# JiaweiXu8/AD-GS

Measured on AMD Instinct MI355X. Metric: fwd+bwd frames/s, higher is better.
Workload: dtype f32; 1 GPU; C3: 1000000 Gaussians, 1920x1280, SH deg 3, 8 dynamic objects, flow+semantic outputs, 1 camera/GPU/step; P=1000000, camera_pool=16 cameras / time stamps per GPU, cycled one per step (train.py:55-61), settle_steps=91, capacity_reruns=0, launch=eager, parallelism=single GPU, gradient_exchange=none, camera_streams=1

## Files before the change

### ad-gs_amd/adgs/_lib.py

```python
import contextlib
import ctypes
import os

_HERE = os.path.dirname(os.path.abspath(__file__))
PKG_ROOT = os.path.dirname(_HERE)
LIB_PATH = os.environ.get("ADGS_LIB") or os.path.join(PKG_ROOT, "lib", "libadgs_hip.so")

ALLOC_FN = ctypes.CFUNCTYPE(ctypes.c_void_p, ctypes.c_void_p, ctypes.c_size_t)

_lib = None

c_p = ctypes.c_void_p
c_i = ctypes.c_int
c_f = ctypes.c_float

SIGNATURES = {
    "adgs_last_error": (ctypes.c_char_p, []),
    "adgs_device_check": (c_i, []),
    "adgs_raster_forward": (c_i, [ALLOC_FN, c_p, ALLOC_FN, c_p, ALLOC_FN, c_p, c_i, c_i, c_i, c_i, c_p, c_i, c_i,
                                  c_p, c_p, c_p, c_p, c_p, c_p, c_p, c_f, c_p, c_p, c_p, c_p, c_p, c_f, c_f, c_i,
                                  c_p, c_p, c_p, c_p, c_p, c_i, c_p, c_i, c_p]),
    "adgs_raster_render": (c_i, [ALLOC_FN, c_p, ALLOC_FN, c_p, ALLOC_FN, c_p, c_i, c_i, c_i, c_i, c_p, c_i, c_i,
                                 c_p, c_p, c_p, c_p, c_p, c_p, c_p, c_f, c_p, c_p, c_p, c_p, c_p, c_f, c_f, c_i,
                                 c_p, c_p, c_p, c_p, c_p, c_i, c_p, c_i, c_p]),
# ... 112 lines not shown
    "adgs_tsdf_extract_count": (c_i, [c_p, c_p, c_p, c_f, c_p, c_p, c_p]),
    "adgs_tsdf_extract_emit": (c_i, [c_p, c_p, c_p, c_p, c_f, c_p, c_p, c_p, c_p, c_p, c_p, c_p]),
    "adgs_mesh_label_temp_bytes": (ctypes.c_size_t, [ctypes.c_longlong, ctypes.c_longlong]),
    "adgs_mesh_label": (c_i, [c_i, c_i, c_p, c_p, c_p, c_p, c_p]),
    "adgs_mesh_table": (c_i, [c_i, c_i, c_i, c_p, c_p, c_p, c_p, c_p, c_p, c_p, c_p, c_p]),
    "adgs_mesh_keep_temp_bytes": (ctypes.c_size_t, [ctypes.c_longlong, ctypes.c_longlong]),
    "adgs_mesh_keep_count": (c_i, [c_i, c_i, c_i, c_p, c_p, c_p, c_p, c_p, c_p]),
    "adgs_mesh_keep_emit": (c_i, [c_i, c_i, c_p, c_p, c_p, c_p, c_p, c_p, c_p, c_p, c_p, c_p, c_p]),
    "adgs_mesh_normals_temp_bytes": (ctypes.c_size_t, [ctypes.c_longlong, ctypes.c_longlong]),
    "adgs_mesh_vertex_normals": (c_i, [c_i, c_i, c_p, c_p, c_p, c_p, c_p]),
    "adgs_test_v2_published_entries": (ctypes.c_longlong, [c_p, c_i, c_i, c_p]),
    "adgs_test_v2_scanned_candidates": (ctypes.c_longlong, [c_p, c_i, c_i, c_p]),
    "adgs_test_v2_tile_counters": (ctypes.c_longlong, [c_p, c_i, c_i, c_p, c_p, ctypes.c_longlong, c_p]),
    "adgs_test_v2_blend_batches": (ctypes.c_longlong, [c_p, c_i, c_i, c_p]),
    "adgs_test_v2_cell_ranges": (ctypes.c_longlong, [c_p, c_i, c_i, c_p, ctypes.c_longlong, c_p]),
    "adgs_test_abi_sizeof": (ctypes.c_size_t, [c_i]),
    "adgs_test_set_capacity_hints": (None, [ctypes.c_longlong, ctypes.c_longlong]),
    "adgs_test_env_reads": (ctypes.c_ulonglong, []),
    "adgs_test_scramble_slab_bounds": (c_i, [ctypes.c_uint]),
    "adgs_test_scan_temp_bytes": (ctypes.c_size_t, [ctypes.c_size_t]),
    "adgs_test_exclusive_scan_u32": (c_i, [c_p, c_p, ctypes.c_size_t, c_p, c_p]),
    "adgs_test_sort_temp_bytes": (ctypes.c_size_t, [ctypes.c_size_t]),
    "adgs_test_sort_pairs_u64": (c_i, [c_p, c_p, c_p, c_p, ctypes.c_size_t, c_i, c_p, c_p]),
    "adgs_test_sort_pairs_u32": (c_i, [c_p, c_p, c_p, c_p, ctypes.c_size_t, c_i, c_p, c_p]),
    "adgs_test_bilagrid_path": (c_i, [c_i, c_i, c_i, c_i, c_i]),
    "adgs_test_deform_plan": (c_i, [c_p, c_i, c_i, c_i, c_p, c_p, c_p, c_p, c_p, c_p, c_p, c_p, c_p, c_p]),
}


class RasterOptions(ctypes.Structure):
# ... 114 lines not shown
```

### ad-gs_amd/csrc/api.hip

```cpp
#include "common.h"
#include "kernels.h"
#include "../../include/adgs_rasterizer.h"
#include "../../include/adgs_optim.h"

#include <atomic>
#include <chrono>
#include <mutex>
#include <vector>
#include <cstdlib>
#include <algorithm>
#include <cmath>
#include <cstring>

namespace adgs {

static thread_local std::string g_last_error;
struct FrameContext {
	adgs_frame_stats stats;
	size_t hint_cells, hint_fine;
	unsigned hint_max_cell_chunks;
	bool bucket_frame_pending;
	long long reruns;
	int last_order_hint;
	uint32_t* slab_bounds;
// ... 53 lines not shown
		b.list_unsorted = c.take<uint32_t>(R);
		b.keys = c.take<uint64_t>(R);
		b.keys_unsorted = c.take<uint64_t>(R);
		b.sort_temp = c.take<char>(sort_temp_bytes(R));
		if (bytes) *bytes = c.size();
		return b;
	}
};

struct GeomStateV2 {
	Splat* splats; uint8_t* clamped; uint32_t* cells_touched; uint32_t* offsets; uint32_t* fine_touched; uint4* dupinfo;
	float* gacc; float* sh0; char* scan_temp; unsigned long long* fine_total;
	float* ddir;
	uint32_t* counters; uint32_t* cell_start; uint2* cell_work; uint32_t* bounds; uint32_t* counts;
	static constexpr size_t COUNTER_WORDS = MAX_CELLS + 2 * SCAN_AUX_SLOTS + 8;
	uint32_t* cell_count() const { return counters; }
	unsigned long long* bucket_fine_total() const { return reinterpret_cast<unsigned long long*>(counters + MAX_CELLS); }
	uint32_t* d_counts() const { return counters + MAX_CELLS + 2 * SCAN_AUX_SLOTS; }
	static GeomStateV2 carve(char* chunk, size_t P, size_t* bytes, bool with_ddir, size_t ncells = 0) {
		Carver c(chunk); GeomStateV2 g;
		g.counters = c.take<uint32_t>(COUNTER_WORDS);
		g.cell_start = c.take<uint32_t>(MAX_CELLS + 1);
		g.cell_work = c.take<uint2>(MAX_CELLS + 1);
		g.splats = c.take<Splat>(P);
		g.gacc = c.take<float>(P * GACC_STRIDE);
		g.dupinfo = c.take<uint4>(P);
		g.clamped = c.take<uint8_t>(P);
		g.cells_touched = c.take<uint32_t>(P + 1);
		g.offsets = c.take<uint32_t>(P + 1);
		g.fine_touched = c.take<uint32_t>(P + 1);
		g.sh0 = c.take<float>(P * 3);
		g.fine_total = c.take<unsigned long long>(SCAN_AUX_SLOTS);
		g.scan_temp = c.take<char>(scan_temp_bytes(P + 1));
		g.ddir = with_ddir ? c.take<float>(P * 9) : nullptr;
		const size_t nc = std::min<size_t>(ncells, (size_t)MAX_CELLS + 1);
		g.bounds = c.take<uint32_t>(nc * SLAB_ROW);
		g.counts = c.take<uint32_t>(count_row_stride((int)((P + 255) / 256)) * nc);
		if (bytes) *bytes = c.size();
		return g;
	}
};
struct ImgStateV2 {
// ... 147 lines not shown
			entries.push_back(fresh);
			e = &entries.back();
		}
		e->view = view; e->proj = proj; e->W = W; e->H = H; e->tiles = tiles; e->stream = stream; e->captured = captured; e->used = ++clock; e->written = false; e->extra = extra;
		if (!reset_signature(e->buf, tiles, extra)) { e->view = nullptr; e->tiles = 0; (void)hipFree(e->buf); e->buf = nullptr; return nullptr; }
		return e;
	}
};
static OrderHints* order_hints() {
	constexpr int MAX_DEV = 64;
	static thread_local OrderHints hints[MAX_DEV];
	int dev = 0;
	if (hipGetDevice(&dev) != hipSuccess || dev < 0 || dev >= MAX_DEV) return nullptr;
	return &hints[dev];
}
struct FrameCfg { int v2; int cell_tiles; int ppl; int tile_order = 1; int sh_staging = 1; int timeline = 0; int order_ready = 0; int backwards = 0; int antialiasing = 0; };
static uint32_t frame_cfg_word(const FrameCfg& c) {
	return 0xAD600000u | ((uint32_t)(c.v2 & 1) << 19) | ((uint32_t)(c.tile_order & 1) << 18) | ((uint32_t)(c.sh_staging & 1) << 17) | ((uint32_t)(c.timeline & 1) << 16) |
	       ((uint32_t)(c.order_ready & 1) << 15) | ((uint32_t)(c.antialiasing & 1) << 14) |
	       ((uint32_t)(c.ppl & 0x3f) << 8) | (uint32_t)(c.cell_tiles & 0xff);
}
static bool frame_cfg_from_word(uint32_t w, FrameCfg* c) {
	if ((w & 0xFFF00000u) != 0xAD600000u) return false;
	*c = FrameCfg{ (int)((w >> 19) & 1u), (int)(w & 0xffu), (int)((w >> 8) & 0x3fu) };
	c->tile_order = (int)((w >> 18) & 1u); c->sh_staging = (int)((w >> 17) & 1u); c->timeline = (int)((w >> 16) & 1u); c->order_ready = (int)((w >> 15) & 1u);
	c->antialiasing = (int)((w >> 14) & 1u);
	return c->cell_tiles >= 1 && (c->ppl == 1 || c->ppl == 2 || c->ppl == 4);
}
struct FrameKey {
	const void* img; const void* geom; int W, H, P;
	bool operator==(const FrameKey& o) const { return img == o.img && geom == o.geom && W == o.W && H == o.H && P == o.P; }
};
static std::mutex g_cfg_mu;
static std::vector<std::pair<FrameKey, FrameCfg>> g_cfg_table;
static void remember_frame(const FrameKey& k, const FrameCfg& c) {
	std::lock_guard<std::mutex> lk(g_cfg_mu);
	for (auto it = g_cfg_table.begin(); it != g_cfg_table.end();) it = (it->first.img == k.img || it->first.geom == k.geom) ? g_cfg_table.erase(it) : it + 1;
	if (g_cfg_table.size() >= 256) g_cfg_table.erase(g_cfg_table.begin());
	g_cfg_table.emplace_back(k, c);
}
static int note_backward(const FrameKey& k) {
// ... 159 lines not shown
		const int wgy = (height + 4 * ppl - 1) / (4 * ppl);
		const size_t wtiles = (size_t)gx * wgy;
		ImgStateV2::carve(nullptr, npix, wtiles, ncells, &ib);
		char* ich = imageBuffer(imageUser, ib);
		if (!gch || !ich) { set_error("buffer allocator returned NULL"); return -1; }
		GeomStateV2 geom = GeomStateV2::carve(gch, P, nullptr, with_ddir, count_cells);
		ImgStateV2 img = ImgStateV2::carve(ich, npix, wtiles, ncells, nullptr);
		uint32_t frame_word = 0; bool order_tiles = false;
		{
			FrameCfg fcfg{ 1, cell_tiles, ppl };
			fcfg.antialiasing = antialiasing ? 1 : 0;
			fcfg.tile_order = env_int("ADGS_TILE_ORDER", 1) != 0; fcfg.sh_staging = env_str("ADGS_NO_SH_STAGING") == nullptr; fcfg.timeline = env_int("ADGS_TIMELINE_BWD", 0) != 0;
			order_tiles = wtiles >= 2048 && fcfg.tile_order;
			if (!training) order_tiles = false;
			fcfg.order_ready = order_tiles ? 1 : 0;
			if (training) remember_frame(FrameKey{ ich, gch, width, height, P }, fcfg);
			frame_word = frame_cfg_word(fcfg);
		}
		const int fwd_order_mode = env_int("ADGS_FWD_ORDER", 2);
		OrderHints::Entry* hint = nullptr;
		const uint32_t* hint_read = nullptr;
		const bool fwd_hint_wanted = wtiles >= 2048 && env_int("ADGS_TILE_ORDER", 1) != 0 && fwd_order_mode == 2;
		if (fwd_hint_wanted) {
			hipStreamCaptureStatus cs0 = hipStreamCaptureStatusNone;
			(void)hipStreamIsCapturing(stream, &cs0);
			if (OrderHints* oh = order_hints()) {
				const bool cap0 = cs0 == hipStreamCaptureStatusActive;
				hint = oh->find(viewmatrix, projmatrix, width, height, wtiles, stream, cap0);
				if (!hint && training) {
					hipStreamCaptureMode mode = hipStreamCaptureModeRelaxed;
// ... 12 lines not shown
		pa.means3D = means3D; pa.scales = scales; pa.scale_modifier = scale_modifier; pa.rotations = rotations;
		pa.opacities = opacities; pa.shs = shs; pa.cov3D_precomp = cov3D_precomp; pa.colors_precomp = colors_precomp;
		pa.flow_points = flow_points; pa.semantic = semantic;
		pa.view = viewmatrix; pa.proj = projmatrix; pa.campos = cam_pos;
		pa.W = width; pa.H = height; pa.gx = gx; pa.gy = gy;
		pa.tan_fovx = tan_fovx; pa.tan_fovy = tan_fovy;
		pa.focal_y = height / (2.0f * tan_fovy); pa.focal_x = width / (2.0f * tan_fovx);
		pa.inv_depth = inv_depth;
		pa.radii = radii; pa.splats = geom.splats; pa.cov3D = nullptr; pa.clamped = geom.clamped; pa.tiles_touched = geom.cells_touched;
		pa.v2 = 1; pa.dupinfo = geom.dupinfo; pa.fine_touched = geom.fine_touched; pa.cell_tiles = cell_tiles; pa.cgx = cgx; pa.cgy = cgy;
		memset(&pa.sh_src, 0, sizeof(pa.sh_src));
		pa.sh0 = geom.sh0; pa.gacc = training ? geom.gacc : nullptr; pa.fine_total = geom.fine_total;
		pa.bucket_count = nullptr;
		pa.cfg_word = img.header; pa.cfg_value = frame_word;
		pa.ddir = geom.ddir;
		pa.antialias = antialiasing ? 1 : 0;
		FramePrologue pro{ nullptr, 0, nullptr, nullptr, 0 };
		bool own_bounds = false, sample_bounds = false;
		if (buckets) {
			if (!fc->slab_bounds) {
				hipStreamCaptureStatus csb = hipStreamCaptureStatusNone;
				(void)hipStreamIsCapturing(stream, &csb);
				hipStreamCaptureMode mode = hipStreamCaptureModeRelaxed;
				if (csb == hipStreamCaptureStatusActive) (void)hipThreadExchangeStreamCaptureMode(&mode);
				bool ok = hipMalloc((void**)&fc->slab_bounds, (size_t)MAX_CELLS * SLAB_ROW * sizeof(uint32_t)) == hipSuccess;
				ok = ok && (fc->service || hipStreamCreateWithFlags(&fc->service, hipStreamNonBlocking) == hipSuccess);
				ok = ok && hipMemsetAsync(fc->slab_bounds, 0xff, (size_t)MAX_CELLS * SLAB_ROW * sizeof(uint32_t), fc->service) == hipSuccess && hipStreamSynchronize(fc->service) == hipSuccess;
				if (csb == hipStreamCaptureStatusActive) (void)hipThreadExchangeStreamCaptureMode(&mode);
				if (!ok) { if (fc->slab_bounds) (void)hipFree(fc->slab_bounds); fc->slab_bounds = nullptr; (void)hipGetLastError(); }
			}
// ... 99 lines not shown
		};
		auto launch_blend = [&]() -> int {
			RenderV2FwdArgs ra;
			ra.cell_ranges = img.cell_ranges; ra.cell_list = bin.list; ra.splats = geom.splats;
			ra.cell_keys = bin.keys; ra.mask_shift = mask_shift; ra.cell_entries = buckets ? bin.entries : nullptr;
			ra.W = width; ra.H = height; ra.gx = gx; ra.gy = wgy; ra.ppl = ppl; ra.cell_tiles = cell_tiles; ra.cgx = cgx;
			ra.has_color = (colors_precomp != nullptr) || (shs != nullptr) || (sh_src != nullptr);
			ra.has_flow = flow_points != nullptr; ra.has_sem = (semantic != nullptr) && D_S > 0;
			ra.bg = background; ra.bg_image = sh_src ? sh_src->bg_image : nullptr;
			ra.pool = bin.pool; ra.pool_cursor = bin.pool_cursor; ra.tile_last_chunk = img.tile_last_chunk; ra.tile_consumed = img.tile_consumed; ra.tile_scanned = img.tile_scanned; ra.tile_batches = img.tile_batches;
			ra.final_T = img_opacity; ra.n_contrib = img.n_contrib;
			ra.out_color = out_color; ra.out_depth = out_depth; ra.out_flow = img_flow; ra.out_semantic = img_semantic;
			ra.order_mode = fwd_order_mode == 2 ? 1 : fwd_order_mode; ra.fwd_order = nullptr;
			ra.fwd_view = viewmatrix; ra.fwd_sig = nullptr;
			if (hint_read) { ra.order_mode = 2; ra.fwd_order = hint_read; ra.fwd_sig = reinterpret_cast<const float*>(hint_read + wtiles); }
			ra.overflow_flag = overflow_flag; ra.publish = training;
			{ StageTimer t(ST_RENDER_FWD, stream);
			  if (launch_render_fwd_v2(ra, stream) != 0) return -1;
			  for (int c0 = 1; ra.has_sem && c0 < D_S; c0 += 4) {
				RenderV2SemFwdArgs sa;
				sa.splats = geom.splats; sa.pool = bin.pool; sa.tile_last_chunk = img.tile_last_chunk; sa.tile_consumed = img.tile_consumed; sa.n_contrib = img.n_contrib;
				sa.W = width; sa.H = height; sa.gx = gx; sa.gy = wgy; sa.ppl = ppl;
				sa.semantic = semantic; sa.D_S = D_S; sa.c0 = c0; sa.nch = std::min(4, D_S - c0); sa.out_semantic = img_semantic;
				if (launch_render_sem_fwd_v2(sa, stream) != 0) return -1;
			  } }
			if (order_tiles) {
				StageTimer t(ST_RENDER_FWD, stream);
				if (launch_tile_order((int)wtiles, img.tile_consumed, img.tile_order, stream, hint ? hint->buf : nullptr, viewmatrix) != 0) return -1;
				if (hint) hint->written = true;
			}
			ADGS_LAUNCH_CHECK(debug, stream);
// ... 61 lines not shown
	PreprocessArgs pa;
	pa.P = P; pa.D = D; pa.M = M; pa.D_S = D_S;
	pa.means3D = means3D; pa.scales = scales; pa.scale_modifier = scale_modifier; pa.rotations = rotations;
	pa.opacities = opacities; pa.shs = shs; pa.cov3D_precomp = cov3D_precomp; pa.colors_precomp = colors_precomp;
	pa.flow_points = flow_points; pa.semantic = semantic;
	pa.view = viewmatrix; pa.proj = projmatrix; pa.campos = cam_pos;
	pa.W = width; pa.H = height; pa.gx = gx; pa.gy = gy;
	pa.tan_fovx = tan_fovx; pa.tan_fovy = tan_fovy;
	pa.focal_y = height / (2.0f * tan_fovy);
	pa.focal_x = width / (2.0f * tan_fovx);
	pa.inv_depth = inv_depth;
	pa.radii = radii; pa.splats = geom.splats; pa.cov3D = geom.cov3D; pa.clamped = geom.clamped; pa.tiles_touched = geom.tiles_touched;
	pa.v2 = 0; pa.dupinfo = nullptr; pa.fine_touched = nullptr; pa.cell_tiles = 1; pa.cgx = gx; pa.cgy = gy;
	memset(&pa.sh_src, 0, sizeof(pa.sh_src)); pa.sh0 = nullptr; pa.gacc = nullptr; pa.fine_total = nullptr;
	pa.bucket_count = nullptr;
	pa.cfg_word = img.header; pa.cfg_value = frame_word; pa.ddir = nullptr;
	pa.antialias = antialiasing ? 1 : 0;
	if (sh_src) { set_error("the raw-SH entry points need the default (v2) pipeline (not ADGS_RASTER_MODE=classic, D_S <= ADGS_V2_MAX_SEMANTIC)"); return -1; }
	{ StageTimer t(ST_PREPROCESS, stream); if (launch_preprocess_fwd(pa, stream) != 0) return -1; }
	ADGS_LAUNCH_CHECK(debug, stream);

	{
		StageTimer t(ST_SCAN, stream);
		if (exclusive_scan_u32(geom.tiles_touched, geom.offsets, (size_t)P + 1, geom.scan_temp, stream) != 0) return -1;
	}
	ADGS_LAUNCH_CHECK(debug, stream);

	uint32_t* host_word = pinned_word();
	if (!host_word) { set_error("hipHostMalloc failed"); return -1; }
	ADGS_HIP_CHECK(hipMemcpyAsync(host_word, geom.offsets + P, sizeof(uint32_t), hipMemcpyDeviceToHost, stream));
	ADGS_HIP_CHECK(hipStreamSynchronize(stream));
// ... 125 lines not shown
		pa.cov3D = cov3D_precomp;
		pa.view = viewmatrix; pa.proj = projmatrix; pa.campos = campos;
		pa.focal_y = height / (2.0f * tan_fovy); pa.focal_x = width / (2.0f * tan_fovx);
		pa.tan_fovx = tan_fovx; pa.tan_fovy = tan_fovy; pa.inv_depth = inv_depth;
		pa.dL_dmean2D = nullptr; pa.dL_dconic = nullptr; pa.dL_dcolor = nullptr; pa.dL_ddepth = nullptr;
		pa.dL_dmean3D = dL_dmean3D; pa.dL_dcov3D = dL_dcov3D; pa.dL_dsh = dL_dsh; pa.dL_dscale = dL_dscale; pa.dL_drot = dL_drot;
		pa.gacc = geom.gacc; pa.splats = geom.splats; pa.W = width; pa.H = height;
		memset(&pa.sh_src, 0, sizeof(pa.sh_src)); pa.sh_dst = ShGradDst{};
		if (sh_src) { pa.sh_src = *sh_src; if (sh_dst) pa.sh_dst = *sh_dst; }
		pa.out_mean2D = dL_dmean2D; pa.out_conic = dL_dconic; pa.out_opacity = dL_dopacity; pa.out_color = dL_dcolor; pa.out_depth = dL_ddepth;
		pa.out_flow = ra.do_flow ? dL_dflow : nullptr; pa.out_sem = ra.do_sem ? dL_dsemantic : nullptr; pa.D_S = D_S;
		pa.out_mean2D_abs = dL_dmean2D_abs;
		pa.sh_staging = cfg.sh_staging;
		pa.ddir = geom.ddir;
		pa.antialias = cfg.antialiasing;
		{ StageTimer t(ST_PREPROCESS_BWD, stream); if (launch_preprocess_bwd(pa, stream) != 0) return -1; }
		ADGS_LAUNCH_CHECK(debug, stream);
		return 0;
	}
	GeomState geom = GeomState::carve(geom_buffer, P, nullptr);
	ImgState img = ImgState::carve(img_buffer, npix, ntiles, nullptr);
	BinState bin = BinState::carve(binning_buffer, (size_t)R, nullptr);

	const bool has_color = (colors_precomp != nullptr) || (shs != nullptr);
	RenderBwdArgs ra;
	ra.ranges = img.ranges; ra.point_list = bin.list; ra.splats = geom.splats;
	ra.W = width; ra.H = height; ra.gx = gx; ra.gy = gy; ra.D_S = D_S;
	ra.semantic = semantic; ra.bg = background;
	ra.final_T = img_opacity; ra.n_contrib = img.n_contrib;
	ra.dL_dpix = dL_dpix; ra.dL_dpix_depth = dL_dpix_depth; ra.dL_dpix_flow = dL_dpix_flow; ra.dL_dpix_sem = dL_dpix_semantic;
// ... 12 lines not shown

	PreprocessBwdArgs pa;
	pa.P = P; pa.D = D; pa.M = M;
	pa.means3D = means3D; pa.radii = radii; pa.shs = shs; pa.clamped = geom.clamped;
	pa.scales = scales; pa.rotations = rotations; pa.scale_modifier = scale_modifier;
	pa.cov3D = cov3D_precomp ? cov3D_precomp : geom.cov3D;
	pa.view = viewmatrix; pa.proj = projmatrix; pa.campos = campos;
	pa.focal_y = height / (2.0f * tan_fovy); pa.focal_x = width / (2.0f * tan_fovx);
	pa.tan_fovx = tan_fovx; pa.tan_fovy = tan_fovy; pa.inv_depth = inv_depth;
	pa.dL_dmean2D = dL_dmean2D; pa.dL_dconic = dL_dconic; pa.dL_dcolor = dL_dcolor; pa.dL_ddepth = dL_ddepth;
	pa.dL_dmean3D = dL_dmean3D; pa.dL_dcov3D = dL_dcov3D; pa.dL_dsh = dL_dsh; pa.dL_dscale = dL_dscale; pa.dL_drot = dL_drot;
	if (sh_src) { set_error("the raw-SH entry points need the default (v2) pipeline (not ADGS_RASTER_MODE=classic, D_S <= ADGS_V2_MAX_SEMANTIC)"); return -1; }
	memset(&pa.sh_src, 0, sizeof(pa.sh_src)); pa.sh_dst = ShGradDst{};
	pa.gacc = nullptr; pa.splats = nullptr; pa.W = width; pa.H = height; pa.out_mean2D = nullptr; pa.out_conic = nullptr; pa.out_opacity = nullptr; pa.out_color = nullptr; pa.out_depth = nullptr;
	pa.out_flow = nullptr; pa.out_sem = nullptr; pa.D_S = D_S; pa.out_mean2D_abs = nullptr;
	pa.sh_staging = cfg.sh_staging; pa.ddir = nullptr;
	pa.antialias = cfg.antialiasing;
	if (cfg.antialiasing) { pa.out_opacity = dL_dopacity; pa.splats = geom.splats; }
	{ StageTimer t(ST_PREPROCESS_BWD, stream); if (launch_preprocess_bwd(pa, stream) != 0) return -1; }
	ADGS_LAUNCH_CHECK(debug, stream);
	return 0;
}

static int read_raster_options(const adgs_raster_options* o, const char* who, int* antialiasing) {
	*antialiasing = 0;
	if (!o) return 0;
	if (o->struct_bytes < offsetof(adgs_raster_options, antialiasing) + sizeof(int32_t) || o->struct_bytes > 4096) {
		set_error(std::string(who) + ": adgs_raster_options.struct_bytes must be sizeof(adgs_raster_options) of the caller's header"); return -1;
	}
	adgs_raster_options full;
	memset(&full, 0, sizeof(full));
// ... 304 lines not shown
}
long long sum_tile_words(const uint32_t* d_words, size_t n, hipStream_t stream) {
	std::vector<uint32_t> h(n);
	if (hipMemcpyAsync(h.data(), d_words, n * sizeof(uint32_t), hipMemcpyDeviceToHost, stream) != hipSuccess) return -1;
	if (hipStreamSynchronize(stream) != hipSuccess) return -1;
	long long total = 0;
	for (uint32_t x : h) total += x;
	return total;
}
}
extern "C" long long adgs_test_v2_published_entries(const char* img_buffer, int width, int height, void* stream_) {
	V2ImageView v;
	if (!v2_image_view(img_buffer, width, height, &v)) return -1;
	return sum_tile_words(v.img.tile_consumed, v.wtiles, (hipStream_t)stream_);
}
extern "C" long long adgs_test_v2_tile_counters(const char* img_buffer, int width, int height, uint32_t* out_consumed, uint32_t* out_scanned, long long capacity, void* stream_) {
	V2ImageView v;
	if (!v2_image_view(img_buffer, width, height, &v)) return -1;
	if ((long long)v.wtiles > capacity) return (long long)v.wtiles;
	if (out_consumed && hipMemcpyAsync(out_consumed, v.img.tile_consumed, v.wtiles * sizeof(uint32_t), hipMemcpyDeviceToHost, (hipStream_t)stream_) != hipSuccess) return -1;
	if (out_scanned && hipMemcpyAsync(out_scanned, v.img.tile_scanned, v.wtiles * sizeof(uint32_t), hipMemcpyDeviceToHost, (hipStream_t)stream_) != hipSuccess) return -1;
	if (hipStreamSynchronize((hipStream_t)stream_) != hipSuccess) return -1;
	return (long long)v.wtiles;
}
extern "C" long long adgs_test_v2_tile_words(const char* img_buffer, int width, int height, uint32_t* out_scanned, uint32_t* out_batches, long long capacity, void* stream_) {
	V2ImageView v;
	if (!v2_image_view(img_buffer, width, height, &v)) return -1;
	if ((long long)v.wtiles > capacity) return (long long)v.wtiles;
	if (out_scanned && hipMemcpyAsync(out_scanned, v.img.tile_scanned, v.wtiles * sizeof(uint32_t), hipMemcpyDeviceToHost, (hipStream_t)stream_) != hipSuccess) return -1;
	if (out_batches && hipMemcpyAsync(out_batches, v.img.tile_batches, v.wtiles * sizeof(uint32_t), hipMemcpyDeviceToHost, (hipStream_t)stream_) != hipSuccess) return -1;
// ... 68 lines not shown
```

### ad-gs_amd/csrc/kernels.h

```cpp
#pragma once
#include "common.h"
#include "func_eval.h"

namespace adgs {

struct PreprocessArgs {
	int P, D, M, D_S;
	const float* means3D; const float* scales; float scale_modifier; const float* rotations;
	const float* opacities; const float* shs; const float* cov3D_precomp; const float* colors_precomp;
	const float* flow_points; const float* semantic;
	const float* view; const float* proj; const float* campos;
	int W, H, gx, gy;
	float tan_fovx, tan_fovy, focal_x, focal_y;
	int inv_depth;
	int* radii; Splat* splats; float* cov3D; uint8_t* clamped; uint32_t* tiles_touched;
	int v2;
	uint32_t* fine_touched;
	uint4* dupinfo;
	int cell_tiles, cgx, cgy;
	ShSource sh_src;
	const float* sh0;
	float* gacc;
	unsigned long long* fine_total;
	uint32_t* bucket_count;
	uint32_t* cfg_word; uint32_t cfg_value;
	float* ddir;
	int antialias;
};

int launch_preprocess_fwd(const PreprocessArgs& a, hipStream_t stream);
int launch_mark_visible(int P, const float* means, const float* view, uint8_t* present, hipStream_t stream);
int launch_duplicate_keys(int P, const Splat* splats, const uint32_t* offsets, const int* radii, uint64_t* keys, uint32_t* vals,
	int gx, int gy, hipStream_t stream);
int launch_tile_ranges(int L, const uint32_t* d_L, const uint64_t* keys, uint2* ranges, uint32_t id_mask, hipStream_t stream);

struct RenderFwdArgs {
	const uint2* ranges; const uint32_t* point_list; const Splat* splats;
	int W, H, gx, gy, D_S;
	bool has_color, has_flow, has_sem, inv_depth;
	const float* semantic;
	const float* bg;
	float* final_T;
// ... 26 lines not shown
	const float* scales; const float* rotations; float scale_modifier;
	const float* cov3D;
	const float* view; const float* proj; const float* campos;
	float focal_x, focal_y, tan_fovx, tan_fovy;
	int inv_depth;
	const float* dL_dmean2D; const float* dL_dconic; const float* dL_dcolor; const float* dL_ddepth;
	float* dL_dmean3D; float* dL_dcov3D; float* dL_dsh; float* dL_dscale; float* dL_drot;
	float* gacc; const Splat* splats; int W, H;
	ShSource sh_src; ShGradDst sh_dst;
	float* out_mean2D; float* out_conic; float* out_opacity; float* out_color; float* out_depth; float* out_flow; float* out_sem;
	float* out_mean2D_abs;
	int D_S;
	int sh_staging;
	const float* ddir;
	int antialias;
};
int launch_preprocess_bwd(const PreprocessBwdArgs& a, hipStream_t stream);

constexpr int CHUNK_WORDS = 2 + WAVE;
constexpr int CHUNK_PREV = WAVE, CHUNK_COUNT = WAVE + 1;
constexpr int POOL_BLOCK = 4;
constexpr int GACC_STRIDE = 16;
constexpr int GACC_USED = 14;

constexpr int MAX_CELLS = 1024;
constexpr int SLAB_ROW = 128;
constexpr int MAX_SLAB_LG = 7;
constexpr int SLAB_TARGET = 3072;
constexpr int SLAB_TARGET_FOREIGN = 2048;
constexpr int GS_NMAX = 4096;
// ... 45 lines not shown
	const uint64_t* cell_keys; int mask_shift;
	const uint2* cell_entries;
	int W, H, gx, gy, cell_tiles, cgx;
	int ppl;
	bool has_color, has_flow, has_sem;
	const float* bg;
	const float* bg_image;
	uint32_t* pool; uint32_t* pool_cursor; uint32_t* tile_last_chunk; uint32_t* tile_consumed; uint32_t* tile_scanned; uint32_t* tile_batches;
	float* final_T; uint32_t* n_contrib;
	float* out_color; float* out_depth; float* out_flow; float* out_semantic;
	int order_mode;
	const uint32_t* fwd_order;
	const float* fwd_view; const float* fwd_sig;
	const uint32_t* overflow_flag;
	bool publish;
};
int launch_render_fwd_v2(const RenderV2FwdArgs& a, hipStream_t stream);

struct RenderV2BwdArgs {
	const Splat* splats; const uint32_t* pool; const uint32_t* tile_last_chunk; const uint32_t* tile_consumed;
	int W, H, gx, gy, ppl;
	const float* bg; const float* final_T; const uint32_t* n_contrib;
	const float* bg_image; float* dL_dbg_image;
	const float* dL_dpix; const float* dL_dpix_depth; const float* dL_dpix_flow; const float* dL_dpix_sem; const float* dL_dpix_opacity;
	bool do_color, do_flow, do_sem, do_depth, do_opacity;
	bool absgrad;
	float* gacc;
	const uint32_t* tile_order;
	uint32_t* tl_start; uint32_t* tl_end;
	const float* sem_src; float* sem_dst; int sem_stride;
// ... 34 lines not shown
```

### ad-gs_amd/csrc/preprocess.hip

```cpp
#include "common.h"
#include "kernels.h"
#include "geom.h"
#include <cstdlib>

#ifndef ADGS_PRE_STAGE_U4
#define ADGS_PRE_STAGE_U4 12
#endif
namespace adgs {

namespace {

struct M3 { float v[3][3]; };

__device__ __forceinline__ M3 m3mul(const M3& a, const M3& b) {
	M3 r;
#pragma unroll
	for (int c = 0; c < 3; c++)
#pragma unroll
		for (int rr = 0; rr < 3; rr++)
			r.v[c][rr] = a.v[0][rr] * b.v[c][0] + a.v[1][rr] * b.v[c][1] + a.v[2][rr] * b.v[c][2];
	return r;
}
__device__ __forceinline__ M3 m3t(const M3& a) {
	M3 r;
// ... 121 lines not shown
			in = load_pre_in(a, idx);
#pragma unroll
			for (int u = 0; u < NQ4; u++) {
				const int q = tid + u * 256;
				if (q < total4) {
					const int g = q / NQ4, c = (q - g * NQ4) * 4;
					float* d = s_sh + g * SH_ROW_FULL_LDS + c;
					d[0] = v[u].x; d[1] = v[u].y; d[2] = v[u].z; d[3] = v[u].w;
				}
			}
		}
	}
	if (STAGED || a.bucket_count) __syncthreads();
	if (a.v2 && !a.bucket_count && idx < SCAN_AUX_SLOTS) a.fine_total[idx] = 0ull;
	PreOut o = { 0u, 0u };
	if (idx < a.P) o = preprocess_one<STAGED, AA>(a, idx, s_sh, s_cell, in);
	if (a.bucket_count) {
		__shared__ uint32_t s_red[256 / WAVE];
		uint32_t nf = o.nfine;
#pragma unroll
		for (int off = WAVE / 2; off > 0; off >>= 1) nf += __shfl_xor(nf, off, WAVE);
		if ((threadIdx.x & (WAVE - 1)) == 0) s_red[threadIdx.x / WAVE] = nf;
		__syncthreads();
		for (int c = threadIdx.x; c < a.cgx * a.cgy; c += 256) a.bucket_count[(size_t)c * count_row_stride((int)gridDim.x) + blockIdx.x] = s_cell[c];
		if (threadIdx.x == 0) {
			uint32_t n = 0;
#pragma unroll
			for (int w = 0; w < 256 / WAVE; w++) n += s_red[w];
			if (n) atomicAdd(a.fine_total + (blockIdx.x & (SCAN_AUX_SLOTS - 1)), (unsigned long long)n);
		}
// ... 293 lines not shown
```

### ad-gs_amd/csrc/preprocess_bwd.hip

```cpp
#include "common.h"
#include "kernels.h"
#include "geom.h"
#include "func_eval.h"
#include <cstdlib>

#ifndef ADGS_PREB_STAGE_U4
#define ADGS_PREB_STAGE_U4 12
#endif
namespace adgs {
namespace {

struct M3 { float v[3][3]; };
__device__ __forceinline__ M3 m3mul(const M3& a, const M3& b) {
	M3 r;
#pragma unroll
	for (int c = 0; c < 3; c++)
#pragma unroll
		for (int rr = 0; rr < 3; rr++)
			r.v[c][rr] = a.v[0][rr] * b.v[c][0] + a.v[1][rr] * b.v[c][1] + a.v[2][rr] * b.v[c][2];
	return r;
}
__device__ __forceinline__ M3 m3t(const M3& a) {
	M3 r;
#pragma unroll
	for (int c = 0; c < 3; c++)
#pragma unroll
		for (int rr = 0; rr < 3; rr++) r.v[c][rr] = a.v[rr][c];
	return r;
}

constexpr int BW_THREADS = 256;
constexpr int SH_ROW_FULL = 48, SH_ROW_FULL_LDS = 49, SH_ROW_REST = 45;

struct PreBIn { alignas(16) float q[4]; float4 u0, u1, u2, u3, s0, s1; float p[3], s[3], op; int radius; uint8_t clamped; float dd[9]; };
__device__ __forceinline__ PreBIn load_preb_in(const PreprocessBwdArgs& a, const int idx) {
	PreBIn in;
	const size_t i = (size_t)min(idx, a.P - 1);
	const bool rs = a.sh_src.scene_xyz != nullptr && (int)i < a.sh_src.Ns;
	in.radius = a.radii[i];
	const float* pos = rs ? a.sh_src.scene_xyz : a.means3D;
	in.p[0] = pos[3 * i]; in.p[1] = pos[3 * i + 1]; in.p[2] = pos[3 * i + 2];
	const float* sc = rs ? a.sh_src.scene_scaling : a.scales;
	const float* rt = rs ? a.sh_src.scene_rotation : a.rotations;
	in.s[0] = sc[3 * i]; in.s[1] = sc[3 * i + 1]; in.s[2] = sc[3 * i + 2];
	const float4 r = *reinterpret_cast<const float4*>(rt + 4 * i);
	in.q[0] = r.x; in.q[1] = r.y; in.q[2] = r.z; in.q[3] = r.w;
	in.op = rs ? a.sh_src.scene_opacity[i] : 0.f;
	const float4* ga = reinterpret_cast<const float4*>(a.gacc + i * GACC_STRIDE);
	in.u0 = ld_stream4(ga); in.u1 = ld_stream4(ga + 1); in.u2 = ld_stream4(ga + 2); in.u3 = ld_stream4(ga + 3);
	const float4* sp = reinterpret_cast<const float4*>(a.splats + i);
	in.s0 = ld_stream4(sp); in.s1 = ld_stream4(sp + 1);
	in.clamped = a.clamped[i];
	if (a.ddir) {
#pragma unroll
		for (int k = 0; k < 9; k++) in.dd[k] = ld_stream(a.ddir + (size_t)k * a.P + i);
	}
	return in;
}

template <bool STAGED, bool AA>
__global__ void __launch_bounds__(BW_THREADS) preprocess_bwd_kernel(PreprocessBwdArgs a) {
	extern __shared__ float s_sh[];
	const int tid = threadIdx.x;
	const int base = blockIdx.x * BW_THREADS;
	const int idx = base + tid;
	const bool raw = a.sh_src.scene_dc != nullptr;
	const int nvalid = min(BW_THREADS, a.P - base);
	const bool pf = STAGED && a.gacc != nullptr && a.cov3D == nullptr && a.scales != nullptr && a.rotations != nullptr;
	const bool adam_rest = STAGED && raw && (a.sh_dst.adam.scene_rest.p != nullptr || a.sh_dst.adam.obj_rest.p != nullptr);
	PreBIn in;
	const bool have_ddir = STAGED && raw && pf && a.ddir != nullptr && a.D == 3;
	if (STAGED) {
		if (raw && have_ddir) {
			in = load_preb_in(a, idx);
		} else if (raw) {
			stage_rows<true, ADGS_PREB_STAGE_U4>(s_sh, SH_ROW_REST, SH_ROW_REST, base, nvalid, a.sh_src.Ns, a.sh_src.scene_rest, a.sh_src.obj_rest, tid, BW_THREADS,
				[&]() { if (pf) in = load_preb_in(a, idx); });
		} else {
			const float4* src = reinterpret_cast<const float4*>(a.shs + (size_t)base * SH_ROW_FULL);
			constexpr int NQ4 = SH_ROW_FULL / 4;
			const int total4 = nvalid * NQ4;
			float4 v[NQ4];
#pragma unroll
			for (int u = 0; u < NQ4; u++) v[u] = ld_stream4(src + min(tid + u * BW_THREADS, total4 - 1));
			if (pf) in = load_preb_in(a, idx);
#pragma unroll
			for (int u = 0; u < NQ4; u++) {
				const int q = tid + u * BW_THREADS;
				if (q < total4) {
					const int g = q / NQ4, c = (q - g * NQ4) * 4;
					float* d = s_sh + g * SH_ROW_FULL_LDS + c;
					d[0] = v[u].x; d[1] = v[u].y; d[2] = v[u].z; d[3] = v[u].w;
				}
			}
		}
		if (!have_ddir) __syncthreads();
	}
	const bool valid = idx < a.P;
	const bool vis = valid && ((pf ? in.radius : a.radii[idx]) > 0);
	const bool rs = a.sh_src.scene_xyz != nullptr && idx < a.sh_src.Ns;
	if (valid && !vis) {
		if (a.gacc) {
			a.out_mean2D[3 * (size_t)idx] = 0.f; a.out_mean2D[3 * (size_t)idx + 1] = 0.f; a.out_mean2D[3 * (size_t)idx + 2] = 0.f;
			if (a.out_mean2D_abs) { a.out_mean2D_abs[3 * (size_t)idx] = 0.f; a.out_mean2D_abs[3 * (size_t)idx + 1] = 0.f; a.out_mean2D_abs[3 * (size_t)idx + 2] = 0.f; }
			if (a.out_conic) *reinterpret_cast<float4*>(a.out_conic + 4 * (size_t)idx) = make_float4(0.f, 0.f, 0.f, 0.f);
			if (!rs) a.out_opacity[idx] = 0.f;
			if (a.out_depth) a.out_depth[idx] = 0.f;
			if (a.out_color) { a.out_color[3 * (size_t)idx] = 0.f; a.out_color[3 * (size_t)idx + 1] = 0.f; a.out_color[3 * (size_t)idx + 2] = 0.f; }
			if (a.out_flow && !rs) { a.out_flow[3 * (size_t)idx] = 0.f; a.out_flow[3 * (size_t)idx + 1] = 0.f; a.out_flow[3 * (size_t)idx + 2] = 0.f; }
			if (a.out_sem && a.D_S >= 1) a.out_sem[(size_t)idx * a.D_S] = 0.f;
			if (rs) {
				float* gx = a.sh_dst.scene_xyz + 3 * (size_t)idx; gx[0] = 0.f; gx[1] = 0.f; gx[2] = 0.f;
				float* gs = a.sh_dst.scene_scaling + 3 * (size_t)idx; gs[0] = 0.f; gs[1] = 0.f; gs[2] = 0.f;
				*reinterpret_cast<float4*>(a.sh_dst.scene_rotation + 4 * (size_t)idx) = make_float4(0.f, 0.f, 0.f, 0.f);
// ... 354 lines not shown
```

### ad-gs_amd/csrc/render_v2.hip

```cpp
#include "common.h"
#include "kernels.h"
#include "blend_instrument.h"
#include <cstdlib>

namespace adgs {
namespace {

constexpr float ALPHA_MAX = 0.99f;
constexpr float ALPHA_MIN = 1.0f / 255.0f;
constexpr float T_STOP = 0.0001f;
constexpr float PIXEL_DONE = 3.0e38f;
constexpr uint32_t NO_CHUNK = 0xFFFFFFFFu;
constexpr int SPLAT_ROW = 5;

#ifndef ADGS_PRECISE_EXP
#define ADGS_EXP2(x) __builtin_amdgcn_exp2f(x)
#else
#define ADGS_EXP2(x) exp2f(x)
#endif
constexpr float LOG2E = 1.4426950408889634f;

__device__ __forceinline__ bool tile_may_contribute(const float4 q0, float C, float tau, uint32_t tx, uint32_t row0, int rows) {
	const float A = q0.z, B = q0.w;
	const float x0 = (float)(tx * TILE_X) - q0.x, x1 = x0 + (float)(TILE_X - 1);
// ... 122 lines not shown
	}
	const int row_bit = (int)(ty16 % a.cell_tiles), col_bit = a.cell_tiles + (int)(tx % a.cell_tiles);
	PT_DECL(10); PT(t_wave0); TL_DECL; PROBE_DECL;

	uint32_t pub_n = 0, pre_block = 0; bool pre_drawn = false;
	auto flush_chunk = [&](uint32_t cnt) {
		if (!PUBLISH) return;
		if (blk_left == 0) {
			if (!pre_drawn) { uint32_t nb = 0; if (lane == 0) nb = atomicAdd(a.pool_cursor, (uint32_t)POOL_BLOCK); pre_block = nb; }
			blk_next = gridDim.x * (uint32_t)POOL_BLOCK + __shfl(pre_block, 0, WAVE); blk_left = POOL_BLOCK; pre_drawn = false;
		}
		const uint32_t chunk = blk_next;
		blk_next++; blk_left--;
		uint32_t* c = a.pool + (size_t)chunk * CHUNK_WORDS;
		const uint32_t mine = s_pub[lane], behind = s_pub[WAVE + lane];
		if ((uint32_t)lane < cnt) c[lane] = mine;
		if (lane == 0) { c[CHUNK_PREV] = prev_chunk; c[CHUNK_COUNT] = cnt; }
		prev_chunk = chunk;
		s_pub[lane] = behind;
		pub_n -= cnt;
	};
	uint32_t entries_in = 0;

	while (true) {
		bool mine_done = true;
#pragma unroll
		for (int k = 0; k < PPL; k++) mine_done = mine_done && (pyf[k] == PIXEL_DONE);
		const bool all_done = !wave_any(!mine_done);
		if (all_done) break;
		__builtin_amdgcn_s_setprio(2);
		PT(t_s1a);
// ... 577 lines not shown
```

### include/adgs_testing.h

```cpp
#ifndef ADGS_TESTING_H
#define ADGS_TESTING_H
#include <stddef.h>
#include <stdint.h>
#include "adgs_deform.h"
#ifdef __cplusplus
extern "C" {
#endif
size_t adgs_test_scan_temp_bytes(size_t n);
int adgs_test_exclusive_scan_u32(const uint32_t* in, uint32_t* out, size_t n, char* temp, void* stream);
size_t adgs_test_sort_temp_bytes(size_t n);
int adgs_test_sort_pairs_u64(uint64_t* keys_in, uint64_t* keys_out, uint32_t* vals_in, uint32_t* vals_out, size_t n, int end_bit, char* temp, void* stream);
int adgs_test_sort_pairs_u32(uint32_t* keys_in, uint32_t* keys_out, uint32_t* vals_in, uint32_t* vals_out, size_t n, int end_bit, char* temp, void* stream);
long long adgs_test_v2_published_entries(const char* img_buffer, int width, int height, void* stream);
long long adgs_test_v2_scanned_candidates(const char* img_buffer, int width, int height, void* stream);
long long adgs_test_v2_tile_counters(const char* img_buffer, int width, int height, uint32_t* out_consumed, uint32_t* out_scanned, long long capacity, void* stream);
long long adgs_test_v2_blend_batches(const char* img_buffer, int width, int height, void* stream);
long long adgs_test_v2_cell_ranges(const char* img_buffer, int width, int height, uint32_t* out_ranges, long long capacity, void* stream);

size_t adgs_test_abi_sizeof(int which);

unsigned long long adgs_test_env_reads(void);

void adgs_test_set_capacity_hints(long long pairs, long long fine_pairs);

int adgs_test_scramble_slab_bounds(unsigned seed);

int adgs_test_bilagrid_path(int L, int Hg, int Wg, int H, int W);

#define ADGS_TEST_DEFORM_PLAN_FIELDS 11
int adgs_test_deform_plan(const adgs_deform_params* p, int np_xyz, int np_xyz_flow, int np_rotation, const adgs_deform_outputs* out, const float* flow_xyz,
	const float* dL_dxyz, const float* dL_drotation, const float* dL_dopacity, const float* dL_dscales, const float* dL_dflow_xyz,
	const adgs_deform_grads* grads, int32_t* fwd, int32_t* bwd);
// ... 6 lines not shown
```

Baseline: 1078 frames/s.

## Gate preprocess backward on a per-Gaussian published mask from forward render

Adds a per-Gaussian byte mask, cleared in preprocess forward and set in the forward render whenever a Gaussian's id is published into a tile chunk. Preprocess backward treats Gaussians never published as invisible and skips loading their full inputs, so Gaussians that passed radius culling but contributed to no pixel do no gradient work. This costs one extra byte write per published entry and a mask read per Gaussian, and it narrows the ppl field in the frame config word. It assumes unpublished Gaussians have zero gradients, so they must get exactly the same handling as the old radius-zero path.

```diff
diff --git a/ad-gs_amd/adgs/_lib.py b/ad-gs_amd/adgs/_lib.py
--- a/ad-gs_amd/adgs/_lib.py
+++ b/ad-gs_amd/adgs/_lib.py
@@ -150,6 +150,8 @@
     "adgs_test_v2_tile_counters": (ctypes.c_longlong, [c_p, c_i, c_i, c_p, c_p, ctypes.c_longlong, c_p]),
     "adgs_test_v2_blend_batches": (ctypes.c_longlong, [c_p, c_i, c_i, c_p]),
     "adgs_test_v2_cell_ranges": (ctypes.c_longlong, [c_p, c_i, c_i, c_p, ctypes.c_longlong, c_p]),
+    "adgs_test_v2_published_mask": (ctypes.c_longlong, [c_p, c_i, c_p, c_p, c_p]),
+    "adgs_test_v2_geom_offsets": (c_i, [c_i, c_p]),
     "adgs_test_abi_sizeof": (ctypes.c_size_t, [c_i]),
     "adgs_test_set_capacity_hints": (None, [ctypes.c_longlong, ctypes.c_longlong]),
     "adgs_test_env_reads": (ctypes.c_ulonglong, []),
diff --git a/ad-gs_amd/csrc/api.hip b/ad-gs_amd/csrc/api.hip
--- a/ad-gs_amd/csrc/api.hip
+++ b/ad-gs_amd/csrc/api.hip
@@ -91,6 +91,7 @@
 	float* ddir;
 	uint32_t* counters; uint32_t* cell_start; uint2* cell_work; uint32_t* bounds; uint32_t* counts;
 	static constexpr size_t COUNTER_WORDS = MAX_CELLS + 2 * SCAN_AUX_SLOTS + 8;
+	uint8_t* published;
 	uint32_t* cell_count() const { return counters; }
 	unsigned long long* bucket_fine_total() const { return reinterpret_cast<unsigned long long*>(counters + MAX_CELLS); }
 	uint32_t* d_counts() const { return counters + MAX_CELLS + 2 * SCAN_AUX_SLOTS; }
@@ -103,6 +104,7 @@
 		g.gacc = c.take<float>(P * GACC_STRIDE);
 		g.dupinfo = c.take<uint4>(P);
 		g.clamped = c.take<uint8_t>(P);
+		g.published = c.take<uint8_t>(P);
 		g.cells_touched = c.take<uint32_t>(P + 1);
 		g.offsets = c.take<uint32_t>(P + 1);
 		g.fine_touched = c.take<uint32_t>(P + 1);
@@ -280,17 +282,17 @@
 	if (hipGetDevice(&dev) != hipSuccess || dev < 0 || dev >= MAX_DEV) return nullptr;
 	return &hints[dev];
 }
-struct FrameCfg { int v2; int cell_tiles; int ppl; int tile_order = 1; int sh_staging = 1; int timeline = 0; int order_ready = 0; int backwards = 0; int antialiasing = 0; };
+struct FrameCfg { int v2; int cell_tiles; int ppl; int tile_order = 1; int sh_staging = 1; int timeline = 0; int order_ready = 0; int backwards = 0; int antialiasing = 0; int published = 0; };
 static uint32_t frame_cfg_word(const FrameCfg& c) {
 	return 0xAD600000u | ((uint32_t)(c.v2 & 1) << 19) | ((uint32_t)(c.tile_order & 1) << 18) | ((uint32_t)(c.sh_staging & 1) << 17) | ((uint32_t)(c.timeline & 1) << 16) |
-	       ((uint32_t)(c.order_ready & 1) << 15) | ((uint32_t)(c.antialiasing & 1) << 14) |
-	       ((uint32_t)(c.ppl & 0x3f) << 8) | (uint32_t)(c.cell_tiles & 0xff);
+	       ((uint32_t)(c.order_ready & 1) << 15) | ((uint32_t)(c.antialiasing & 1) << 14) | ((uint32_t)(c.published & 1) << 13) |
+	       ((uint32_t)(c.ppl & 0x1f) << 8) | (uint32_t)(c.cell_tiles & 0xff);
 }
 static bool frame_cfg_from_word(uint32_t w, FrameCfg* c) {
 	if ((w & 0xFFF00000u) != 0xAD600000u) return false;
-	*c = FrameCfg{ (int)((w >> 19) & 1u), (int)(w & 0xffu), (int)((w >> 8) & 0x3fu) };
+	*c = FrameCfg{ (int)((w >> 19) & 1u), (int)(w & 0xffu), (int)((w >> 8) & 0x1fu) };
 	c->tile_order = (int)((w >> 18) & 1u); c->sh_staging = (int)((w >> 17) & 1u); c->timeline = (int)((w >> 16) & 1u); c->order_ready = (int)((w >> 15) & 1u);
-	c->antialiasing = (int)((w >> 14) & 1u);
+	c->antialiasing = (int)((w >> 14) & 1u); c->published = (int)((w >> 13) & 1u);
 	return c->cell_tiles >= 1 && (c->ppl == 1 || c->ppl == 2 || c->ppl == 4);
 }
 struct FrameKey {
@@ -480,6 +482,7 @@
 			order_tiles = wtiles >= 2048 && fcfg.tile_order;
 			if (!training) order_tiles = false;
 			fcfg.order_ready = order_tiles ? 1 : 0;
+			fcfg.published = (training && env_int("ADGS_PUBLISHED_MASK", 1) != 0) ? 1 : 0;
 			if (training) remember_frame(FrameKey{ ich, gch, width, height, P }, fcfg);
 			frame_word = frame_cfg_word(fcfg);
 		}
@@ -522,6 +525,7 @@
 		pa.bucket_count = nullptr;
 		pa.cfg_word = img.header; pa.cfg_value = frame_word;
 		pa.ddir = geom.ddir;
+		pa.published = training ? geom.published : nullptr;
 		pa.antialias = antialiasing ? 1 : 0;
 		FramePrologue pro{ nullptr, 0, nullptr, nullptr, 0 };
 		bool own_bounds = false, sample_bounds = false;
@@ -651,7 +655,7 @@
 			ra.order_mode = fwd_order_mode == 2 ? 1 : fwd_order_mode; ra.fwd_order = nullptr;
 			ra.fwd_view = viewmatrix; ra.fwd_sig = nullptr;
 			if (hint_read) { ra.order_mode = 2; ra.fwd_order = hint_read; ra.fwd_sig = reinterpret_cast<const float*>(hint_read + wtiles); }
-			ra.overflow_flag = overflow_flag; ra.publish = training;
+			ra.overflow_flag = overflow_flag; ra.publish = training; ra.published = training ? geom.published : nullptr;
 			{ StageTimer t(ST_RENDER_FWD, stream);
 			  if (launch_render_fwd_v2(ra, stream) != 0) return -1;
 			  for (int c0 = 1; ra.has_sem && c0 < D_S; c0 += 4) {
@@ -743,7 +747,7 @@
 	pa.v2 = 0; pa.dupinfo = nullptr; pa.fine_touched = nullptr; pa.cell_tiles = 1; pa.cgx = gx; pa.cgy = gy;
 	memset(&pa.sh_src, 0, sizeof(pa.sh_src)); pa.sh0 = nullptr; pa.gacc = nullptr; pa.fine_total = nullptr;
 	pa.bucket_count = nullptr;
-	pa.cfg_word = img.header; pa.cfg_value = frame_word; pa.ddir = nullptr;
+	pa.cfg_word = img.header; pa.cfg_value = frame_word; pa.ddir = nullptr; pa.published = nullptr;
 	pa.antialias = antialiasing ? 1 : 0;
 	if (sh_src) { set_error("the raw-SH entry points need the default (v2) pipeline (not ADGS_RASTER_MODE=classic, D_S <= ADGS_V2_MAX_SEMANTIC)"); return -1; }
 	{ StageTimer t(ST_PREPROCESS, stream); if (launch_preprocess_fwd(pa, stream) != 0) return -1; }
@@ -899,6 +903,7 @@
 		pa.sh_staging = cfg.sh_staging;
 		pa.ddir = geom.ddir;
 		pa.antialias = cfg.antialiasing;
+		pa.published = cfg.published ? geom.published : nullptr;
 		{ StageTimer t(ST_PREPROCESS_BWD, stream); if (launch_preprocess_bwd(pa, stream) != 0) return -1; }
 		ADGS_LAUNCH_CHECK(debug, stream);
 		return 0;
@@ -941,7 +946,7 @@
 	memset(&pa.sh_src, 0, sizeof(pa.sh_src)); pa.sh_dst = ShGradDst{};
 	pa.gacc = nullptr; pa.splats = nullptr; pa.W = width; pa.H = height; pa.out_mean2D = nullptr; pa.out_conic = nullptr; pa.out_opacity = nullptr; pa.out_color = nullptr; pa.out_depth = nullptr;
 	pa.out_flow = nullptr; pa.out_sem = nullptr; pa.D_S = D_S; pa.out_mean2D_abs = nullptr;
-	pa.sh_staging = cfg.sh_staging; pa.ddir = nullptr;
+	pa.sh_staging = cfg.sh_staging; pa.ddir = nullptr; pa.published = nullptr;
 	pa.antialias = cfg.antialiasing;
 	if (cfg.antialiasing) { pa.out_opacity = dL_dopacity; pa.splats = geom.splats; }
 	{ StageTimer t(ST_PREPROCESS_BWD, stream); if (launch_preprocess_bwd(pa, stream) != 0) return -1; }
@@ -1276,6 +1281,21 @@
 	if (!v2_image_view(img_buffer, width, height, &v)) return -1;
 	return sum_tile_words(v.img.tile_consumed, v.wtiles, (hipStream_t)stream_);
 }
+extern "C" long long adgs_test_v2_published_mask(const char* geom_buffer, int P, uint8_t* out_bytes, float* out_lines, void* stream_) {
+	if (!geom_buffer || P <= 0) return -1;
+	const GeomStateV2 g = GeomStateV2::carve(const_cast<char*>(geom_buffer), (size_t)P, nullptr, false);
+	if (out_bytes && hipMemcpyAsync(out_bytes, g.published, (size_t)P, hipMemcpyDeviceToHost, (hipStream_t)stream_) != hipSuccess) return -1;
+	if (out_lines && hipMemcpyAsync(out_lines, g.gacc, (size_t)P * GACC_STRIDE * sizeof(float), hipMemcpyDeviceToHost, (hipStream_t)stream_) != hipSuccess) return -1;
+	if (hipStreamSynchronize((hipStream_t)stream_) != hipSuccess) return -1;
+	return (long long)P;
+}
+extern "C" int adgs_test_v2_geom_offsets(int P, long long* out2) {
+	if (P <= 0 || !out2) return -1;
+	char* const base = reinterpret_cast<char*>((uintptr_t)1 << 20);
+	const GeomStateV2 g = GeomStateV2::carve(base, (size_t)P, nullptr, false);
+	out2[0] = (long long)(reinterpret_cast<char*>(g.published) - base); out2[1] = (long long)(reinterpret_cast<char*>(g.gacc) - base);
+	return 0;
+}
 extern "C" long long adgs_test_v2_tile_counters(const char* img_buffer, int width, int height, uint32_t* out_consumed, uint32_t* out_scanned, long long capacity, void* stream_) {
 	V2ImageView v;
 	if (!v2_image_view(img_buffer, width, height, &v)) return -1;
diff --git a/ad-gs_amd/csrc/kernels.h b/ad-gs_amd/csrc/kernels.h
--- a/ad-gs_amd/csrc/kernels.h
+++ b/ad-gs_amd/csrc/kernels.h
@@ -26,6 +26,7 @@
 	uint32_t* cfg_word; uint32_t cfg_value;
 	float* ddir;
 	int antialias;
+	uint8_t* published;
 };
 
 int launch_preprocess_fwd(const PreprocessArgs& a, hipStream_t stream);
@@ -82,6 +83,7 @@
 	int sh_staging;
 	const float* ddir;
 	int antialias;
+	const uint8_t* published;
 };
 int launch_preprocess_bwd(const PreprocessBwdArgs& a, hipStream_t stream);
 
@@ -157,6 +159,7 @@
 	const float* fwd_view; const float* fwd_sig;
 	const uint32_t* overflow_flag;
 	bool publish;
+	uint8_t* published;
 };
 int launch_render_fwd_v2(const RenderV2FwdArgs& a, hipStream_t stream);
 
diff --git a/ad-gs_amd/csrc/preprocess.hip b/ad-gs_amd/csrc/preprocess.hip
--- a/ad-gs_amd/csrc/preprocess.hip
+++ b/ad-gs_amd/csrc/preprocess.hip
@@ -159,6 +159,7 @@
 	if (STAGED || a.bucket_count) __syncthreads();
 	if (a.v2 && !a.bucket_count && idx < SCAN_AUX_SLOTS) a.fine_total[idx] = 0ull;
 	PreOut o = { 0u, 0u };
+	if (idx < a.P && a.published) a.published[idx] = (uint8_t)0;
 	if (idx < a.P) o = preprocess_one<STAGED, AA>(a, idx, s_sh, s_cell, in);
 	if (a.bucket_count) {
 		__shared__ uint32_t s_red[256 / WAVE];
diff --git a/ad-gs_amd/csrc/preprocess_bwd.hip b/ad-gs_amd/csrc/preprocess_bwd.hip
--- a/ad-gs_amd/csrc/preprocess_bwd.hip
+++ b/ad-gs_amd/csrc/preprocess_bwd.hip
@@ -33,11 +33,12 @@
 constexpr int SH_ROW_FULL = 48, SH_ROW_FULL_LDS = 49, SH_ROW_REST = 45;
 
 struct PreBIn { alignas(16) float q[4]; float4 u0, u1, u2, u3, s0, s1; float p[3], s[3], op; int radius; uint8_t clamped; float dd[9]; };
-__device__ __forceinline__ PreBIn load_preb_in(const PreprocessBwdArgs& a, const int idx) {
+__device__ __forceinline__ PreBIn load_preb_in(const PreprocessBwdArgs& a, const int idx, const bool gate, const bool pub) {
 	PreBIn in;
 	const size_t i = (size_t)min(idx, a.P - 1);
 	const bool rs = a.sh_src.scene_xyz != nullptr && (int)i < a.sh_src.Ns;
-	in.radius = a.radii[i];
+	in.radius = gate ? 0 : a.radii[i];
+	if (!pub) return in;
 	const float* pos = rs ? a.sh_src.scene_xyz : a.means3D;
 	in.p[0] = pos[3 * i]; in.p[1] = pos[3 * i + 1]; in.p[2] = pos[3 * i + 2];
 	const float* sc = rs ? a.sh_src.scene_scaling : a.scales;
@@ -68,14 +69,17 @@
 	const int nvalid = min(BW_THREADS, a.P - base);
 	const bool pf = STAGED && a.gacc != nullptr && a.cov3D == nullptr && a.scales != nullptr && a.rotations != nullptr;
 	const bool adam_rest = STAGED && raw && (a.sh_dst.adam.scene_rest.p != nullptr || a.sh_dst.adam.obj_rest.p != nullptr);
+	const bool gate = a.gacc != nullptr && a.published != nullptr;
+	bool pub = true;
+	if (gate) pub = idx < a.P && a.published[idx] != 0;
 	PreBIn in;
 	const bool have_ddir = STAGED && raw && pf && a.ddir != nullptr && a.D == 3;
 	if (STAGED) {
 		if (raw && have_ddir) {
-			in = load_preb_in(a, idx);
+			in = load_preb_in(a, idx, gate, pub);
 		} else if (raw) {
 			stage_rows<true, ADGS_PREB_STAGE_U4>(s_sh, SH_ROW_REST, SH_ROW_REST, base, nvalid, a.sh_src.Ns, a.sh_src.scene_rest, a.sh_src.obj_rest, tid, BW_THREADS,
-				[&]() { if (pf) in = load_preb_in(a, idx); });
+				[&]() { if (pf) in = load_preb_in(a, idx, gate, pub); });
 		} else {
 			const float4* src = reinterpret_cast<const float4*>(a.shs + (size_t)base * SH_ROW_FULL);
 			constexpr int NQ4 = SH_ROW_FULL / 4;
@@ -83,7 +87,7 @@
 			float4 v[NQ4];
 #pragma unroll
 			for (int u = 0; u < NQ4; u++) v[u] = ld_stream4(src + min(tid + u * BW_THREADS, total4 - 1));
-			if (pf) in = load_preb_in(a, idx);
+			if (pf) in = load_preb_in(a, idx, gate, pub);
 #pragma unroll
 			for (int u = 0; u < NQ4; u++) {
 				const int q = tid + u * BW_THREADS;
@@ -97,7 +101,7 @@
 		if (!have_ddir) __syncthreads();
 	}
 	const bool valid = idx < a.P;
-	const bool vis = valid && ((pf ? in.radius : a.radii[idx]) > 0);
+	const bool vis = valid && (gate ? pub : (pf ? in.radius : a.radii[idx]) > 0);
 	const bool rs = a.sh_src.scene_xyz != nullptr && idx < a.sh_src.Ns;
 	if (valid && !vis) {
 		if (a.gacc) {
diff --git a/ad-gs_amd/csrc/render_v2.hip b/ad-gs_amd/csrc/render_v2.hip
--- a/ad-gs_amd/csrc/render_v2.hip
+++ b/ad-gs_amd/csrc/render_v2.hip
@@ -160,7 +160,10 @@
 		blk_next++; blk_left--;
 		uint32_t* c = a.pool + (size_t)chunk * CHUNK_WORDS;
 		const uint32_t mine = s_pub[lane], behind = s_pub[WAVE + lane];
-		if ((uint32_t)lane < cnt) c[lane] = mine;
+		if ((uint32_t)lane < cnt) {
+			c[lane] = mine;
+			a.published[mine] = (uint8_t)1;
+		}
 		if (lane == 0) { c[CHUNK_PREV] = prev_chunk; c[CHUNK_COUNT] = cnt; }
 		prev_chunk = chunk;
 		s_pub[lane] = behind;
diff --git a/include/adgs_testing.h b/include/adgs_testing.h
--- a/include/adgs_testing.h
+++ b/include/adgs_testing.h
@@ -16,6 +16,8 @@
 long long adgs_test_v2_tile_counters(const char* img_buffer, int width, int height, uint32_t* out_consumed, uint32_t* out_scanned, long long capacity, void* stream);
 long long adgs_test_v2_blend_batches(const char* img_buffer, int width, int height, void* stream);
 long long adgs_test_v2_cell_ranges(const char* img_buffer, int width, int height, uint32_t* out_ranges, long long capacity, void* stream);
+long long adgs_test_v2_published_mask(const char* geom_buffer, int P, uint8_t* out_bytes, float* out_lines, void* stream);
+int adgs_test_v2_geom_offsets(int P, long long* out2);
 
 size_t adgs_test_abi_sizeof(int which);
 
```

Result: faster. 1093 frames/s (median of 6 runs) (+1.3%).
